# batmanlab/Mammo-CLIP

Measured on AMD Instinct MI355X. Metric: image-text pairs/s (whole node), EN-B5+BioClinicalBERT contrastive pre-training step, higher is better.
Workload: dtype bf16; 1 GPU; cfg4: efficientnet-b5 + BioClinicalBERT(BERT-base), 1024 pairs/GPU (2 views + 2 reports each), 1520x912 images, 256-token reports, breast_clip loss, AdamW; fwd+loss+bwd+optimizer; dropout/drop-connect on; global_batch=1024, parallelism=dp1 x 32 micro-batches, keep_graphs=7, recompute=0, keep_recompute=2, stat_tapes=True, streams=3

## Files before the change

include/mammoclip_hip.h:

```cpp
#ifndef MAMMOCLIP_HIP_H
#define MAMMOCLIP_HIP_H
#include <stdint.h>
#ifdef __cplusplus
extern "C" {
#endif

typedef uint16_t mc_bf16;

const char* mc_last_error(void);
int mc_version(void);
int mc_storage_is_f16(void);

typedef struct mc_gemm_args {
    const mc_bf16* A;
    const mc_bf16* B;
    void* C;
    long long M, K;
    int N;
    long long lda, ldb, ldc;
    int a_kmajor, b_kmajor;
    int c_f32, c_atomic;
    int splits;
    int batch, nb2;
    long long sA1, sA2, sB1, sB2, sC1, sC2;
// ... 57 lines not shown
    const float* epi_coef;
    const float* epi_mul;
    const float* epi_add;
    float epi_add_scale;
    float* epi_sums;
    float* epi_ws;
} mc_gemm_rows_args;
int mc_gemm_rows_supported(int n, int k);
long long mc_gemm_rows_epi_ws_floats(const mc_gemm_rows_args* args);
int mc_gemm_rows_epi_supported(long long M, int N, int K, long long rows_per_img, int epi_mode);
int mc_gemm_rows_blocks(const mc_gemm_rows_args* args);
int mc_gemm_rows_bf16(const mc_gemm_rows_args* args, void* stream);

typedef struct mc_wgrad_rows_args {
    const mc_bf16* dY;
    int N;
    long long lddy;
    const mc_bf16* X;
    int K;
    long long ldx;
    long long M;
    float* dW;
    float* ws;
    int accumulate;
    const float* pro_scale;
    const float* pro_shift;
    const float* pro_gate;
    long long pro_rows_per_img;
} mc_wgrad_rows_args;
int mc_wgrad_rows_supported(int n, int k);
int mc_wgrad_rows_blocks(long long m);
int mc_wgrad_rows_bf16(const mc_wgrad_rows_args* args, void* stream);
int mc_xbwd_rows_supported(int n, int k);
int mc_xbwd_rows_blocks(long long m);
int mc_xbwd_rows_bf16(const mc_wgrad_rows_args* args, const mc_bf16* wt, long long ldwt, mc_bf16* dx, long long lddx,
                      const mc_bf16* r, long long ldr, void* stream);

int mc_cast_f32_bf16(const float* src, mc_bf16* dst, long long n, void* stream);
int mc_cast_f32_bf16_lo(const float* src, mc_bf16* dst, long long n, void* stream);
int mc_cast_bf16_f32(const mc_bf16* src, float* dst, long long n, void* stream);
int mc_transpose_f32(const float* src, float* dst, int rows, int cols, void* stream);
int mc_cast_transpose_f32_bf16(const float* src, mc_bf16* dst, int rows, int cols, void* stream);
int mc_stem_weight_prep(const float* w, mc_bf16* out, int c0, void* stream);

int mc_stem_im2col(const float* x, long long sn, long long sc, long long sh, long long sw,
                   int n, int h, int w, int pad_l, int pad_t, int oh, int ow, mc_bf16* out, void* stream);
int mc_gate_weights_bf16(const mc_bf16* w, const float* gate, int n_img, int n, int k, mc_bf16* out, void* stream);

int mc_image_minmax_u8(const unsigned char* x, long long sn, long long elems_per_image, int n,
                       unsigned int* minmax, void* stream);
int mc_stem_im2col_u8(const unsigned char* x, long long sn, long long sc, long long sh, long long sw,
                      const unsigned int* minmax, float mean, float std, int n, int h, int w, int pad_l,
                      int pad_t, int oh, int ow, mc_bf16* out, void* stream);

typedef struct mc_dwconv_args {
    const mc_bf16* x;
    const mc_bf16* dy;
    void* out;
    const float* w_kkc;
    int n, h, w, c;
    int k, stride, pad_l, pad_t, oh, ow;
    const float* pro_scale;
    const float* pro_shift;
    float* stat_partials;
    const mc_bf16* epi_x;
    const float* epi_scale;
    const float* epi_shift;
    const float* epi_mean;
    const float* epi_invstd;
    float* dw_out;
    int stat_rows;
    const mc_bf16* xw;
    int cin;
    float* dw_partials;
    int dw_rows;
} mc_dwconv_args;
int mc_dwconv_stat_rows(const mc_dwconv_args* args);
int mc_dwconv_bwd_data_stat_rows(const mc_dwconv_args* args);
int mc_dwconv_fwd(const mc_dwconv_args* args, void* stream);
int mc_dwconv_bwd_data(const mc_dwconv_args* args, void* stream);
int mc_dwconv_bwd_weight(const mc_dwconv_args* args, void* stream);
int mc_dwconv_bwd_weight_dw_rows(const mc_dwconv_args* args);
int mc_dwconv_bwd_data_dw_rows(const mc_dwconv_args* args);
int mc_dwconv_bwd_fused_dw_rows(const mc_dwconv_args* args);
int mc_dwconv_bwd_data_xw_supported(const mc_dwconv_args* args);
int mc_dwconv_bwd_data_plan(const mc_dwconv_args* args, int* plan);
int mc_dwconv_bwd_data_xw_preferred(const mc_dwconv_args* args);
int mc_dwconv_set_lane_mode(int mode);
int mc_dwconv_lane_supported(const mc_dwconv_args* args);
int mc_dwconv_bwd_fused_supported(const mc_dwconv_args* args);
int mc_dwconv_bwd_fused_preferred(const mc_dwconv_args* args);
int mc_dwconv_bwd_fused_stat_rows(const mc_dwconv_args* args);
int mc_dwconv_bwd_fused(const mc_dwconv_args* args, void* stream);
int mc_mbconv_xdw_supported(const mc_dwconv_args* args);
int mc_mbconv_xdw_stat_rows(const mc_dwconv_args* args);
int mc_mbconv_xdw_fwd(const mc_dwconv_args* args, void* stream);

int mc_bn_finalize(const float* partials, int rows, int c, double count, const float* gamma,
                   const float* beta, float* running_mean, float* running_var, float momentum, float eps,
                   int update_running, float* mean, float* invstd, float* scale, float* shift, void* stream);
int mc_bn_eval_coeffs(const float* gamma, const float* beta, const float* running_mean,
                      const float* running_var, float eps, int c, float* scale, float* shift, void* stream);
int mc_bn_eval_stats(const float* gamma, const float* beta, const float* running_mean, const float* running_var,
                     float eps, int c, float* mean, float* invstd, float* scale, float* shift, void* stream);

typedef struct mc_bnact_args {
// ... 199 lines not shown
```

mammo_clip_amd/breastclip/model/modules/efficientnet_custom.py:

```python
import math
from collections import namedtuple
from typing import List, Optional

import os

import torch
from torch import nn

from .... import ops

BN_MOMENTUM = 0.01
BN_EPS = 1e-3

VALID_MODELS = tuple(f"efficientnet-b{i}" for i in range(9)) + ("efficientnet-l2",)

_COEFFS = {
    "efficientnet-b0": (1.0, 1.0, 224, 0.2), "efficientnet-b1": (1.0, 1.1, 240, 0.2),
    "efficientnet-b2": (1.1, 1.2, 260, 0.3), "efficientnet-b3": (1.2, 1.4, 300, 0.3),
    "efficientnet-b4": (1.4, 1.8, 380, 0.4), "efficientnet-b5": (1.6, 2.2, 456, 0.4),
    "efficientnet-b6": (1.8, 2.6, 528, 0.5), "efficientnet-b7": (2.0, 3.1, 600, 0.5),
    "efficientnet-b8": (2.2, 3.6, 672, 0.5), "efficientnet-l2": (4.3, 5.3, 800, 0.5),
}
_STAGES = ((1, 3, 1, 1, 32, 16), (2, 3, 2, 6, 16, 24), (2, 5, 2, 6, 24, 40), (3, 3, 2, 6, 40, 80),
           (3, 5, 1, 6, 80, 112), (4, 5, 2, 6, 112, 192), (1, 3, 1, 6, 192, 320))
# ... 99 lines not shown
            return
        if self.flat.is_cuda:
            self.flat.record_stream(torch.cuda.current_stream(self.flat.device))
        dst = [bn.running_mean for bn in self.used] + [bn.running_var for bn in self.used]
        src = [self.flat[self.offs[id(bn)]:self.offs[id(bn)] + bn.num_features] for bn in self.used] + \
              [self.flat[self.total + self.offs[id(bn)]:self.total + self.offs[id(bn)] + bn.num_features] for bn in self.used]
        torch._foreach_mul_(dst, 1.0 - BN_MOMENTUM)
        torch._foreach_add_(dst, src)
        self.used = []


_BN_DEFER = None


def _bn_stats(partials, count, bn: nn.BatchNorm2d, training: bool):
    if training:
        if _replaying():
            return _TAPE.get()
        if _BN_DEFER is not None and bn.track_update:
            rm, rv = _BN_DEFER.scratch(bn)
        else:
            rm, rv = bn.running_mean, bn.running_var
        st = ops.bn_finalize(partials, count, bn.weight, bn.bias, rm, rv, BN_MOMENTUM, BN_EPS, bn.track_update)
        if bn.track_update:
            if bn.defer_count is not None:
                bn.defer_count.append(bn.num_batches_tracked)
            else:
                bn.num_batches_tracked += 1
        if _TAPE is not None:
            _TAPE.put(st)
        return st
    return ops.bn_eval_coeffs(bn.weight, bn.bias, bn.running_mean, bn.running_var, BN_EPS)


def _conv_stats(fn, training, *a, stats=True, **kw):
    if not stats or (training and _replaying()):
        return fn(*a, **kw), None
    return fn(*a, stats=True, **kw)


def _no_fp8_frozen(mod):
    if mod.fp8:
        raise NotImplementedError("backward through BatchNorm on running statistics (eval mode / freeze_bn) is not implemented "
                                  "for the fp8 forward (set_fp8)")


LINK_STEM = os.environ.get("MC_LINK_STEM", "1") != "0"
FUSE_DW_BWD = os.environ.get("MC_FUSE_DW_BWD", "1") != "0"
FUSE_PROJ_DGRAD = os.environ.get("MC_FUSE_PROJ_DGRAD", "1") != "0"
BN_FOLD_MIN_BYTES = int(os.environ.get("MC_BN_FOLD_MIN_BYTES", 250_000_000))
BN_FOLD_S2_MIN_BYTES = int(os.environ.get("MC_BN_FOLD_S2_MIN_BYTES", 0))
XDW_MAX_CIN = int(os.environ.get("MC_XDW_MAX_CIN", 64))
MODE3_MAX_CEXP = int(os.environ.get("MC_MODE3_MAX_CEXP", 1 << 30))


class _StemFn(torch.autograd.Function):

    @staticmethod
    def forward(ctx, x, w, gamma, beta, mod, link=None):
        n, _, h, wd = x.shape
        l, r, t, b = mod.stem_pad
        _, oh, ow = mod.stem_geo(n, h, wd)
        c0 = w.shape[0]
        patches = ops.stem_im2col(x, l, t, oh, ow)
        wb = ops.stem_weight_prep(w)
        training = mod.batch_stats
        e, part = _conv_stats(ops.linear_fwd, training, patches, wb)
        st = _bn_stats(part, n * oh * ow, mod._bn0, training)
        ctx.mod, ctx.st, ctx.geo, ctx.frozen = mod, st, (n, h, wd, oh, ow, c0), not training
        ctx.raw = (x.mean, x.std) if isinstance(x, ops.RawImages) else None
        ctx.save_for_backward(x.data if ctx.raw else x, e)
        ctx.link = link
        if link is not None:
            link.st, link.part = st, None
            return e.detach()
        return ops.bnact_apply(e, n, oh * ow, c0, st.scale, st.shift, 1)

    @staticmethod
    def backward(ctx, dy):
        x, e = ctx.saved_tensors
        if ctx.raw:
            x = ops.RawImages(x, *ctx.raw)
        n, h, wd, oh, ow, c0 = ctx.geo
        mod = ctx.mod
        link = ctx.link
        if ctx.frozen:
            _no_fp8_frozen(mod)
        if ctx.frozen and link is not None:
            de = dy.contiguous()
            _, dgamma, dbeta = ops.bn_bwd_coefs(link.part, 0, ctx.st, mod._bn0.weight, frozen=True)
            link.part = None
        elif ctx.frozen:
            de, dgamma, dbeta = ops.bnact_bwd(e, n, oh * ow, c0, ctx.st, mod._bn0.weight, 1, g=dy.contiguous(), frozen=True)
        elif link is not None:
            de, dgamma, dbeta = ops.bnact_bwd(e, n, oh * ow, c0, ctx.st, mod._bn0.weight, 0, g=dy.contiguous(), partials=link.part)
            link.part = None
        else:
            de, dgamma, dbeta = ops.bnact_bwd(e, n, oh * ow, c0, ctx.st, mod._bn0.weight, 1, g=dy.contiguous())
        l, r, t, b = mod.stem_pad
        patches = ops.stem_im2col(x, l, t, oh, ow)
        dw = ops.linear_wgrad(de, patches)
        if ctx.frozen and link is not None:
            dw = ops.rowscale_f32_(dw, ctx.st.scale)
        gw, gg, gb = ops.deliver_param_grads((mod._conv_stem.weight, mod._bn0.weight, mod._bn0.bias),
                                             (dw[:, :27].reshape(c0, 3, 3, 3), dgamma, dbeta))
        return (None, gw, gg, gb, None) + ((None,) if link is not None else ())


class _StemLink:
    __slots__ = ("st", "part")

    def __init__(self):
        self.st, self.part = None, None


def _expand_conv(pl, x, we, stats=True):
    if pl.fp8_expand:
        return ops.linear_fwd_fp8(x, we, stats=True)
    return _conv_stats(ops.linear_fwd, pl.batch_stats, x, we, stats=stats)


def _depthwise(blk, pl, x, e, we, wkkc, pro0, stats=True):
    if pl.xdw:
        return _conv_stats(ops.mbconv_xdw_fwd, pl.batch_stats, x, we, pro0, wkkc, *pl.dw, stats=stats)
    return _conv_stats(ops.dwconv_fwd, pl.batch_stats, e if blk.args.expand != 1 else x, wkkc, *pl.dw, stats=stats, pro=pro0)


def _project_conv(pl, d, act1, st1, gate, wp, stats=True):
    ohw = pl.oh * pl.ow
    if pl.fp8_project:
        wg = ops.gate_weights(wp, gate)
        return ops.linear_fwd_fp8(act1, wg, stats=True, batch_w=(pl.n, ohw))
    src, pro = (act1, (None, None, gate, ohw)) if pl.keep_act else (d, (st1.scale, st1.shift, gate, ohw))
    return _conv_stats(ops.linear_fwd, pl.batch_stats, src, wp, stats=stats, pro=pro)


class _MBConvFn(torch.autograd.Function):

    @staticmethod
    def forward(ctx, x, rowscale, blk, n, h, w, recording, link, *params):
        a = blk.args
        pl = blk.plan(n, h, w, recording)
        training, bstat, ohw = pl.training, pl.batch_stats, pl.oh * pl.ow
        wkkc = blk.w_taps()
        e = we = st0 = gram = None
        if a.expand != 1:
            we = blk.w_expand()
            if pl.xdw:
                if bstat and _replaying():
                    part0, gram = None, _TAPE.get()
                elif bstat:
                    part0, gram = ops.bn_gram_partials(x, we, n * h * w)
# ... 598 lines not shown
```

mammo_clip_amd/lib.py:

```python
import ctypes as C
import os

_HERE = os.path.dirname(os.path.abspath(__file__))
STORAGE = os.environ.get("MC_STORAGE", "bf16").lower()
if STORAGE not in ("bf16", "f16"):
    raise ValueError(f"MC_STORAGE must be 'bf16' or 'f16', got {STORAGE!r}")
LIB_PATH = os.path.join(_HERE, "lib", "libmammoclip_hip.so" if STORAGE == "bf16" else "libmammoclip_hip_f16.so")

P, LL, I, F, D, U, ULL = C.c_void_p, C.c_longlong, C.c_int, C.c_float, C.c_double, C.c_uint, C.c_ulonglong


class GemmArgs(C.Structure):
    _fields_ = [
        ("A", P), ("B", P), ("C", P),
        ("M", LL), ("K", LL), ("N", I),
        ("lda", LL), ("ldb", LL), ("ldc", LL),
        ("a_kmajor", I), ("b_kmajor", I),
        ("c_f32", I), ("c_atomic", I),
        ("splits", I),
        ("batch", I), ("nb2", I),
        ("sA1", LL), ("sA2", LL), ("sB1", LL), ("sB2", LL), ("sC1", LL), ("sC2", LL),
        ("bias", P), ("bias_stride1", LL),
        ("act", I),
        ("R", P), ("ldr", LL),
# ... 52 lines not shown
        ("scale", P), ("shift", P), ("act", I),
        ("rowscale", P), ("res", P), ("out", P),
        ("pooled", P),
        ("g", P), ("mul", P), ("add", P), ("add_scale", F), ("mean", P), ("invstd", P),
        ("partials", P), ("coef", P), ("dx", P), ("dgate", P), ("split_ws", P),
    ]


class AdamwTensor(C.Structure):
    _fields_ = [("param", P), ("grad", P), ("exp_avg", P), ("exp_avg_sq", P), ("numel", LL), ("bf16_image", P)]


_SIGS = {
    "mc_version": ([], I),
    "mc_storage_is_f16": ([], I),
    "mc_adamw_step": ([C.POINTER(AdamwTensor), I, D, D, D, D, D, LL, P], I),
    "mc_grads_unscale": ([C.POINTER(AdamwTensor), I, F, P, P], I),
    "mc_grads_unscale_dev": ([C.POINTER(AdamwTensor), I, P, P, P], I),
    "mc_adamw_step_ls": ([C.POINTER(AdamwTensor), I, D, D, D, D, D, LL, P, P, P], I),
    "mc_loss_scale_update": ([P, P, D, D, I, I, P], I),
    "mc_grad_norm_partials": ([C.POINTER(AdamwTensor), I], LL),
    "mc_grad_norm": ([C.POINTER(AdamwTensor), I, P, LL, F, P, P], I),
    "mc_grads_unscale_norm_dev": ([C.POINTER(AdamwTensor), I, P, P, P, LL, F, P, P], I),
    "mc_grads_scale_dev": ([C.POINTER(AdamwTensor), I, P, P], I),
    "mc_adamw_step_clip": ([C.POINTER(AdamwTensor), I, D, D, D, D, D, LL, P, P, P, P], I),
    "mc_gemm_bf16": ([C.POINTER(GemmArgs), P], I),
    "mc_gemm_stat_rows": ([C.POINTER(GemmArgs)], I),
    "mc_gemm_tile_config": ([C.POINTER(GemmArgs)], I),
    "mc_gemm256_tn_eligible": ([C.POINTER(GemmArgs)], I),
    "mc_gemm256_tn_splits": ([LL, LL, LL, LL], I),
    "mc_amax_bf16": ([P, LL, P, P], I),
    "mc_quant_fp8_bf16": ([P, LL, P, P, P, P, P], I),
    "mc_gemm_rows_supported": ([I, I], I),
    "mc_gemm_rows_blocks": ([C.POINTER(GemmRowsArgs)], I),
    "mc_gemm_rows_epi_ws_floats": ([C.POINTER(GemmRowsArgs)], LL),
    "mc_gemm_rows_epi_supported": ([LL, I, I, LL, I], I),
    "mc_gemm_rows_bf16": ([C.POINTER(GemmRowsArgs), P], I),
    "mc_cast_transpose_f32_bf16": ([P, P, I, I, P], I),
    "mc_wgrad_rows_supported": ([I, I], I),
    "mc_wgrad_rows_blocks": ([LL], I),
    "mc_wgrad_rows_bf16": ([C.POINTER(WgradRowsArgs), P], I),
    "mc_xbwd_rows_supported": ([I, I], I),
    "mc_xbwd_rows_blocks": ([LL], I),
    "mc_xbwd_rows_bf16": ([C.POINTER(WgradRowsArgs), P, LL, P, LL, P, LL, P], I),
    "mc_cast_f32_bf16": ([P, P, LL, P], I),
    "mc_cast_bf16_f32": ([P, P, LL, P], I),
    "mc_cast_f32_bf16_lo": ([P, P, LL, P], I),
    "mc_transpose_f32": ([P, P, I, I, P], I),
    "mc_stem_weight_prep": ([P, P, I, P], I),
    "mc_stem_im2col": ([P, LL, LL, LL, LL, I, I, I, I, I, I, I, P, P], I),
    "mc_image_minmax_u8": ([P, LL, LL, I, P, P], I),
    "mc_gate_weights_bf16": ([P, P, I, I, I, P, P], I),
    "mc_stem_im2col_u8": ([P, LL, LL, LL, LL, P, F, F, I, I, I, I, I, I, I, P, P], I),
    "mc_dwconv_stat_rows": ([C.POINTER(DwconvArgs)], I),
    "mc_dwconv_bwd_data_stat_rows": ([C.POINTER(DwconvArgs)], I),
    "mc_dwconv_fwd": ([C.POINTER(DwconvArgs), P], I),
    "mc_dwconv_bwd_data": ([C.POINTER(DwconvArgs), P], I),
    "mc_dwconv_bwd_data_xw_supported": ([C.POINTER(DwconvArgs)], I),
    "mc_dwconv_bwd_data_plan": ([C.POINTER(DwconvArgs), C.POINTER(C.c_int)], I),
    "mc_dwconv_bwd_data_xw_preferred": ([C.POINTER(DwconvArgs)], I),
    "mc_dwconv_bwd_weight": ([C.POINTER(DwconvArgs), P], I),
    "mc_dwconv_bwd_weight_dw_rows": ([C.POINTER(DwconvArgs)], I),
    "mc_dwconv_bwd_data_dw_rows": ([C.POINTER(DwconvArgs)], I),
    "mc_dwconv_bwd_fused_dw_rows": ([C.POINTER(DwconvArgs)], I),
    "mc_dwconv_set_lane_mode": ([I], I),
    "mc_dwconv_lane_supported": ([C.POINTER(DwconvArgs)], I),
    "mc_dwconv_bwd_fused_supported": ([C.POINTER(DwconvArgs)], I),
    "mc_dwconv_bwd_fused_preferred": ([C.POINTER(DwconvArgs)], I),
    "mc_dwconv_bwd_fused_stat_rows": ([C.POINTER(DwconvArgs)], I),
    "mc_dwconv_bwd_fused": ([C.POINTER(DwconvArgs), P], I),
    "mc_mbconv_xdw_supported": ([C.POINTER(DwconvArgs)], I),
    "mc_mbconv_xdw_stat_rows": ([C.POINTER(DwconvArgs)], I),
    "mc_mbconv_xdw_fwd": ([C.POINTER(DwconvArgs), P], I),
    "mc_bn_gram_partials": ([P, I, P, P, D, I, I, P, P], I),
    "mc_bn_finalize": ([P, I, I, D, P, P, P, P, F, F, I, P, P, P, P, P], I),
    "mc_bn_eval_coeffs": ([P, P, P, P, F, I, P, P, P], I),
    "mc_bn_eval_stats": ([P, P, P, P, F, I, P, P, P, P, P], I),
    "mc_bnact_rows": ([C.POINTER(BnactArgs)], I),
    "mc_bnact_img_splits": ([C.POINTER(BnactArgs)], I),
    "mc_bnact_apply": ([C.POINTER(BnactArgs), P], I),
    "mc_bnact_pool": ([C.POINTER(BnactArgs), P], I),
    "mc_bnact_bwd_reduce": ([C.POINTER(BnactArgs), P], I),
    "mc_bnact_bwd_apply": ([C.POINTER(BnactArgs), P], I),
    "mc_bnact_bwd_frozen": ([C.POINTER(BnactArgs), P], I),
    "mc_bnact_se_dgate": ([C.POINTER(BnactArgs), P], I),
    "mc_bnact_se_sums": ([C.POINTER(BnactArgs), P], I),
    "mc_bn_partials_from_se_sums": ([P, P, P, F, LL, I, P, P], I),
    "mc_bn_bwd_finalize": ([P, I, I, D, P, P, P, P, P, P, P], I),
    "mc_bn_bwd_finalize_frozen": ([P, I, I, P, P, P, P, P], I),
    "mc_bn_frozen_rows": ([P, P, I, I, P, P, P], I),
    "mc_colsum_rows": ([LL, I], I),
    "mc_colsum_bf16": ([P, LL, I, LL, P, P, I, P], I),
    "mc_se_fwd": ([P, P, P, P, P, I, I, I, P, P, P], I),
    "mc_se_bwd": ([P, P, P, P, P, P, P, I, I, I, P, P, P, P, P, P, P], I),
    "mc_dropout_f32": ([P, P, LL, F, ULL, U, P], I),
    "mc_bert_embed_fwd": ([P, P, P, P, P, P, P, F, I, I, I, F, ULL, U, P, P, P, P], I),
    "mc_bert_embed_bwd": ([P, P, P, P, P, P, P, P, P, I, I, I, F, ULL, U, P, P, P, P, P, P], I),
    "mc_add_ln_fwd": ([P, P, P, P, F, LL, I, F, ULL, U, P, P, P, P], I),
    "mc_add_ln_bwd": ([P, P, P, P, P, P, LL, I, F, ULL, U, P, P, P, P, P], I),
    "mc_add_ln_bwd_ws_rows": ([LL], I),
    "mc_add_ln_bwd_ws": ([P, P, P, P, P, P, LL, I, F, ULL, U, P, P, P, P, P, I, P], I),
    "mc_bert_embed_bwd_ws_floats": ([I, I, I, LL, C.POINTER(C.c_int)], LL),
    "mc_bert_embed_bwd_ws": ([P, P, P, P, P, P, P, P, P, I, I, I, F, ULL, U, P, P, P, P, P, P, P, P, LL, P], I),
    "mc_ordered_sum": ([P, I, LL, LL, P, I, P], I),
    "mc_softmax_fwd": ([P, LL, I, F, ULL, U, P, P, P], I),
    "mc_softmax_bwd": ([P, P, LL, I, F, ULL, U, F, P, P], I),
# ... 122 lines not shown
```

mammo_clip_amd/ops.py:

```python
import ctypes as C
import math
import os

import weakref

import torch

from . import lib as L

BF16 = torch.bfloat16 if L.STORAGE == "bf16" else torch.float16


def _p(t):
    return None if t is None else t.data_ptr()


_RAW_STREAM = getattr(torch._C, "_cuda_getCurrentRawStream", None)
_GET_DEV = getattr(torch._C, "_cuda_getDevice", None)


def _st():
    if _RAW_STREAM is None or _GET_DEV is None:
        return torch.cuda.current_stream().cuda_stream
    return _RAW_STREAM(_GET_DEV())
# ... 497 lines not shown
        return dst
    return _cached("t", src, make) if cache else make()


def stem_weight_prep(w):
    c0 = w.shape[0]
    out = empty((c0, 32), BF16, w)
    L.call("mc_stem_weight_prep", _p(w.contiguous()), _p(out), c0, _st())
    return out


class RawImages:

    def __init__(self, data, mean, std):
        assert data.dtype == torch.uint8 and data.dim() == 4 and data.shape[1] == 3, "RawImages: uint8 [b,3,H,W]"
        self.data, self.mean, self.std = data, float(mean), float(std)

    def to(self, device, **kw):
        return RawImages(self.data.to(device, **kw), self.mean, self.std)

    shape = property(lambda self: self.data.shape)
    device = property(lambda self: self.data.device)
    is_cuda = property(lambda self: self.data.is_cuda)
    dtype = property(lambda self: self.data.dtype)


def image_minmax_u8(x):
    n = x.shape[0]
    per = x[0].numel()
    dense = sorted(zip(x.stride()[1:], x.shape[1:]), reverse=True)
    run = 1
    for st, sz in reversed(dense):
        assert sz == 1 or st == run, "RawImages: every image must be one dense block of bytes"
        run *= sz
    mm = torch.empty((2, n), dtype=torch.int32, device=x.device)
    L.call("mc_image_minmax_u8", _p(x), x.stride(0), per, n, _p(mm), _st())
    return mm


def stem_im2col(x, pad_l, pad_t, oh, ow):
    n, c, h, w = x.shape
    if isinstance(x, RawImages):
        d = x.data
        out = empty((n * oh * ow, 32), BF16, d)
        sn, sc, sh, sw = d.stride()
        L.call("mc_stem_im2col_u8", _p(d), sn, sc, sh, sw, _p(image_minmax_u8(d)), x.mean, x.std, n, h, w, pad_l, pad_t,
               oh, ow, _p(out), _st())
        return out
    assert c == 3 and x.dtype == torch.float32
    out = empty((n * oh * ow, 32), BF16, x)
    sn, sc, sh, sw = x.stride()
    L.call("mc_stem_im2col", _p(x), sn, sc, sh, sw, n, h, w, pad_l, pad_t, oh, ow, _p(out), _st())
    return out


def _dw_args(n, h, w, c, k, stride, pad_l, pad_t, oh, ow):
    a = L.DwconvArgs()
    a.n, a.h, a.w, a.c, a.k, a.stride, a.pad_l, a.pad_t, a.oh, a.ow = n, h, w, c, k, stride, pad_l, pad_t, oh, ow
    return a


def _dwconv_fwd_impl(x, w_kkc, n, h, w, c, k, stride, pad_l, pad_t, oh, ow, pro=None, stats=False, epi=None):
    a = _dw_args(n, h, w, c, k, stride, pad_l, pad_t, oh, ow)
    y = empty((n * oh * ow, c), BF16, x)
    a.x, a.out, a.w_kkc = _p(x), _p(y), _p(w_kkc)
    if pro is not None:
        a.pro_scale, a.pro_shift = _p(pro[0]), _p(pro[1])
    if epi is not None:
        e, st = epi
        assert stride == 1 and e.shape == y.shape
        a.epi_x, a.epi_scale, a.epi_shift, a.epi_mean, a.epi_invstd = _p(e), _p(st.scale), _p(st.shift), _p(st.mean), _p(st.invstd)
        stats = True
    part = None
    if stats:
        rows = L.load().mc_dwconv_stat_rows(C.byref(a))
        part = empty((rows, 2, c), torch.float32, x)
        a.stat_partials, a.stat_rows = _p(part), rows
    _note(2 * n * c * (h * w + oh * ow * (2 if epi is not None else 1)), 2 * n * c * oh * ow * k * k)
    L.call("mc_dwconv_fwd", C.byref(a), _st(), kind=f"k{k}s{stride}" + ("|dgrad_bn" if epi is not None else ""))
    return (y, part) if stats else y


def _dwconv_bwd_data_impl(dy, w_kkc, n, h, w, c, k, stride, pad_l, pad_t, oh, ow, w_kkc_flipped=None, epi=None, xw=None, dw=False):
    if stride == 1 and w_kkc_flipped is not None:
        assert xw is None and not dw
        return _dwconv_fwd_impl(dy, w_kkc_flipped, n, oh, ow, c, k, 1, k - 1 - pad_l, k - 1 - pad_t, h, w, epi=epi)
    assert epi is None or stride == 2
    if xw is not None:
        x, we = xw
        assert epi is not None and x.is_contiguous() and we.is_contiguous() and we.shape == (c, x.shape[1]) and x.shape[0] == n * h * w
        cin, st = x.shape[1], epi[1]
        a = _dw_args(n, h, w, c, k, stride, pad_l, pad_t, oh, ow)
        dz = empty((n * h * w, c), BF16, dy)
        a.dy, a.out, a.w_kkc = _p(dy), _p(dz), _p(w_kkc)
        a.epi_x, a.epi_scale, a.epi_shift, a.epi_mean, a.epi_invstd = _p(x), _p(st.scale), _p(st.shift), _p(st.mean), _p(st.invstd)
        a.xw, a.cin = _p(we), cin
        rows = L.load().mc_dwconv_bwd_data_stat_rows(C.byref(a))
        part = empty((rows, 2, c), torch.float32, dy)
        a.stat_partials, a.stat_rows = _p(part), rows
        dwdw = None
        if dw:
            dwdw = torch.zeros((k * k, c), dtype=torch.float32, device=dy.device)
            a.dw_out = _p(dwdw)
            ws = _dw_partials(a, "mc_dwconv_bwd_data_dw_rows", dy)
        _note(2 * n * (c * (oh * ow + h * w) + cin * h * w), (4 if dw else 2) * n * c * oh * ow * k * k + 2 * n * h * w * c * cin)
        L.call("mc_dwconv_bwd_data", C.byref(a), _st(), kind=f"k{k}s{stride}|dgrad_bn|x")
# ... 931 lines not shown
```

Before: 127.3 image-text pairs/s.

## Add direct stem convolution kernels fusing im2col, GEMM, BN stats and wgrad

Adds dedicated HIP kernels for the EfficientNet stem conv. The forward kernel loads image tiles (float or raw uint8 with normalisation) into LDS, runs MFMA against the weights and writes output plus BN statistic partials without materialising an im2col patch buffer. The backward kernel folds the BN-backward coefficients into a weight-gradient computation (dz·X and X·X Gram terms), so the separate bnact_bwd, im2col recompute and wgrad GEMM are skipped. By default the direct forward runs only outside training capture, while the direct backward runs whenever the BN is linked. This adds a multi-kernel reduction path and more numerical complexity in exchange.

```diff
diff --git a/include/mammoclip_hip.h b/include/mammoclip_hip.h
--- a/include/mammoclip_hip.h
+++ b/include/mammoclip_hip.h
@@ -133,6 +133,17 @@
 int mc_stem_im2col_u8(const unsigned char* x, long long sn, long long sc, long long sh, long long sw,
                       const unsigned int* minmax, float mean, float std, int n, int h, int w, int pad_l,
                       int pad_t, int oh, int ow, mc_bf16* out, void* stream);
+
+int mc_stem_conv_blocks(int n, int oh, int ow);
+int mc_stem_conv_set_max_blocks(int blocks);
+long long mc_stem_conv_bwd_ws_floats(int n, int oh, int ow, int c0);
+int mc_stem_conv_fwd(const void* x, int x_u8, long long sn, long long sc, long long sh, long long sw,
+                     const unsigned int* minmax, float mean, float std, int n, int h, int w, int pad_l, int pad_t,
+                     int oh, int ow, const mc_bf16* wimg, int c0, mc_bf16* e, float* stat_partials, void* stream);
+int mc_stem_conv_bwd(const void* x, int x_u8, long long sn, long long sc, long long sh, long long sw,
+                     const unsigned int* minmax, float mean, float std, int n, int h, int w, int pad_l, int pad_t,
+                     int oh, int ow, const mc_bf16* dz, const mc_bf16* wimg, const float* coef, int c0, float* ws,
+                     float* dw, void* stream);
 
 typedef struct mc_dwconv_args {
     const mc_bf16* x;
diff --git a/mammo_clip_amd/breastclip/model/modules/efficientnet_custom.py b/mammo_clip_amd/breastclip/model/modules/efficientnet_custom.py
--- a/mammo_clip_amd/breastclip/model/modules/efficientnet_custom.py
+++ b/mammo_clip_amd/breastclip/model/modules/efficientnet_custom.py
@@ -175,6 +175,7 @@
 BN_FOLD_S2_MIN_BYTES = int(os.environ.get("MC_BN_FOLD_S2_MIN_BYTES", 0))
 XDW_MAX_CIN = int(os.environ.get("MC_XDW_MAX_CIN", 64))
 MODE3_MAX_CEXP = int(os.environ.get("MC_MODE3_MAX_CEXP", 1 << 30))
+STEM_DIRECT = {"0": False, "1": True}.get(os.environ.get("MC_STEM_DIRECT", "1"), "all")
 
 
 class _StemFn(torch.autograd.Function):
@@ -185,12 +186,16 @@
         l, r, t, b = mod.stem_pad
         _, oh, ow = mod.stem_geo(n, h, wd)
         c0 = w.shape[0]
-        patches = ops.stem_im2col(x, l, t, oh, ow)
         wb = ops.stem_weight_prep(w)
         training = mod.batch_stats
-        e, part = _conv_stats(ops.linear_fwd, training, patches, wb)
+        direct = bool(STEM_DIRECT) and 24 <= c0 <= 64 and c0 % 8 == 0
+        if direct and (STEM_DIRECT == "all" or not (training and not _replaying())):
+            e, part = _conv_stats(ops.stem_conv_fwd, training, x, wb, l, t, oh, ow)
+        else:
+            e, part = _conv_stats(ops.linear_fwd, training, ops.stem_im2col(x, l, t, oh, ow), wb)
         st = _bn_stats(part, n * oh * ow, mod._bn0, training)
         ctx.mod, ctx.st, ctx.geo, ctx.frozen = mod, st, (n, h, wd, oh, ow, c0), not training
+        ctx.wb = wb if direct else None
         ctx.raw = (x.mean, x.std) if isinstance(x, ops.RawImages) else None
         ctx.save_for_backward(x.data if ctx.raw else x, e)
         ctx.link = link
@@ -209,6 +214,14 @@
         link = ctx.link
         if ctx.frozen:
             _no_fp8_frozen(mod)
+        l, r, t, b = mod.stem_pad
+        if ctx.wb is not None and link is not None:
+            coef, dgamma, dbeta = ops.bn_bwd_coefs(link.part, 0 if ctx.frozen else n * oh * ow, ctx.st, mod._bn0.weight, frozen=ctx.frozen)
+            link.part = None
+            dw = ops.stem_conv_bwd(x, dy.contiguous(), ctx.wb, coef, l, t, oh, ow)
+            gw, gg, gb = ops.deliver_param_grads((mod._conv_stem.weight, mod._bn0.weight, mod._bn0.bias),
+                                                 (dw[:, :27].reshape(c0, 3, 3, 3), dgamma, dbeta))
+            return (None, gw, gg, gb, None, None)
         if ctx.frozen and link is not None:
             de = dy.contiguous()
             _, dgamma, dbeta = ops.bn_bwd_coefs(link.part, 0, ctx.st, mod._bn0.weight, frozen=True)
@@ -220,7 +233,6 @@
             link.part = None
         else:
             de, dgamma, dbeta = ops.bnact_bwd(e, n, oh * ow, c0, ctx.st, mod._bn0.weight, 1, g=dy.contiguous())
-        l, r, t, b = mod.stem_pad
         patches = ops.stem_im2col(x, l, t, oh, ow)
         dw = ops.linear_wgrad(de, patches)
         if ctx.frozen and link is not None:
diff --git a/mammo_clip_amd/csrc/stem.hip b/mammo_clip_amd/csrc/stem.hip
--- /dev/null
+++ b/mammo_clip_amd/csrc/stem.hip
@@ -0,0 +1,449 @@
+#include "common_hip.h"
+#include "../../include/mammoclip_hip.h"
+
+namespace {
+
+typedef __attribute__((ext_vector_type(4))) short s4_t;
+typedef __attribute__((ext_vector_type(8))) short s8_t;
+typedef __attribute__((address_space(3))) s4_t lds_s4_t;
+
+constexpr int TW = 64, TR = 4;
+constexpr int IR = 2 * TR + 1;
+constexpr int IW = 2 * TW + 1;
+constexpr int PS = TW + 8;
+constexpr int NPL = IR * 9;
+constexpr int PL_ZERO = NPL, PL_ONE = NPL + 1;
+constexpr int SX_ELEMS = (NPL + 2) * PS;
+constexpr int RE = IW * 3;
+constexpr int NH = (RE + 255) / 256;
+constexpr int NLD = IR * NH;
+constexpr int MAX_BLOCKS = 768;
+
+struct stem_geo {
+    const void* x;
+    long long sn, sc, sh, sw;
+    int n, h, w, pad_l, pad_t, oh, ow, c0;
+    const unsigned int* mm;
+    float mean, stdv;
+    int tx, ty;
+    int ntiles;
+};
+
+struct tile_pos { long long img; int oy0, ox0; };
+__device__ __forceinline__ tile_pos tile_of(const stem_geo& g, int t) {
+    tile_pos q;
+    const unsigned t2 = (unsigned)t / (unsigned)g.tx, im = t2 / (unsigned)g.ty;
+    q.ox0 = (int)((unsigned)t - t2 * (unsigned)g.tx) * TW;
+    q.img = im;
+    q.oy0 = (int)(t2 - im * (unsigned)g.ty) * TR;
+    return q;
+}
+
+template <typename SRC>
+__device__ __forceinline__ void stem_load(const stem_geo& g, const tile_pos& q, int tid, SRC (&v)[NLD]) {
+    const int ix0 = q.ox0 * 2 - g.pad_l, iy0 = q.oy0 * 2 - g.pad_t;
+    const SRC* base = reinterpret_cast<const SRC*>(g.x) + q.img * g.sn;
+#pragma unroll
+    for (int hf = 0; hf < NH; ++hf) {
+        const int e = tid + hf * 256, ixl = e / 3, c = e - ixl * 3, ix = ix0 + ixl;
+        const int ixc = ix < 0 ? 0 : (ix < g.w ? ix : g.w - 1);
+        const long long xo = c * g.sc + ixc * g.sw;
+#pragma unroll
+        for (int r = 0; r < IR; ++r) {
+            const int iy = iy0 + r, iyc = iy < 0 ? 0 : (iy < g.h ? iy : g.h - 1);
+            v[r * NH + hf] = base[iyc * g.sh + xo];
+        }
+    }
+}
+
+template <typename SRC, bool MASK>
+__device__ __forceinline__ void stem_store(const stem_geo& g, const tile_pos& q, int tid, const SRC (&v)[NLD], bf16_t* sX) {
+    const int pvalid = MASK ? g.ow - q.ox0 : TW;
+    const int ix0 = q.ox0 * 2 - g.pad_l, iy0 = q.oy0 * 2 - g.pad_t;
+    float lo = 0.f, range = 1.f;
+    if constexpr (sizeof(SRC) == 1) {
+        lo = (float)g.mm[q.img];
+        range = (float)g.mm[g.n + q.img] - lo;
+    }
+#pragma unroll
+    for (int hf = 0; hf < NH; ++hf) {
+        const int e = tid + hf * 256, ixl = e / 3, c = e - ixl * 3, ix = ix0 + ixl;
+        const bool okx = ix >= 0 && ix < g.w;
+        const int p = ixl >> 1;
+        bf16_t* d0 = sX + c * 3 * PS + ((ixl & 1) ? PS + p : p);
+        bf16_t* d2 = sX + c * 3 * PS + 2 * PS + p - 1;
+        const bool w0 = e < RE && ((ixl & 1) || p < TW), w2 = e < RE && !(ixl & 1) && p >= 1;
+        const bool z0 = p >= pvalid, z2 = p - 1 >= pvalid;
+#pragma unroll
+        for (int r = 0; r < IR; ++r) {
+            const int iy = iy0 + r;
+            float val;
+            if constexpr (sizeof(SRC) == 1) {
+                float tt = (float)v[r * NH + hf] - lo;
+                tt = __fdiv_rn(tt, range);
+                val = __fdiv_rn(__fsub_rn(tt, g.mean), g.stdv);
+            } else {
+                val = v[r * NH + hf];
+            }
+            const bf16_t b = (okx && iy >= 0 && iy < g.h) ? f2bf(val) : (bf16_t)0;
+            if (w0) d0[r * 9 * PS] = z0 ? (bf16_t)0 : b;
+            if (w2) d2[r * 9 * PS] = z2 ? (bf16_t)0 : b;
+        }
+    }
+}
+
+__device__ __forceinline__ int plane_of(int k, int row, int pad27) {
+    if (k > 27) return PL_ZERO;
+    if (k == 27) return pad27;
+    const int cin = k / 9, kh = (k - cin * 9) / 3, kw = k - cin * 9 - kh * 3;
+    return (2 * row + kh) * 9 + cin * 3 + kw;
+}
+
+__device__ __forceinline__ bf16x8_t tr_read(const void* lo_addr, const void* hi_addr) {
+    const s4_t lo = __builtin_amdgcn_ds_read_tr16_b64_v4i16((lds_s4_t*)(lo_addr));
+    const s4_t hi = __builtin_amdgcn_ds_read_tr16_b64_v4i16((lds_s4_t*)(hi_addr));
+    const s8_t v = {lo[0], lo[1], lo[2], lo[3], hi[0], hi[1], hi[2], hi[3]};
+    return __builtin_bit_cast(bf16x8_t, v);
+}
+
+template <typename SRC, int FN>
+__global__ __launch_bounds__(256, 3) void stem_conv_fwd_k(const stem_geo g, const bf16_t* __restrict__ wimg, bf16_t* __restrict__ out,
+                                                       float* __restrict__ part) {
+    constexpr int NP = FN * 16, CROW = (NP + 8) * 2;
+    __shared__ __attribute__((aligned(16))) bf16_t sX[SX_ELEMS];
+    __shared__ __attribute__((aligned(16))) unsigned char sC[4 * 16 * CROW];
+    const int tid = threadIdx.x, lane = tid & 63, wave = tid >> 6;
+    const int li = lane & 15, kg = lane >> 4;
+    if (tid < PS) sX[PL_ZERO * PS + tid] = (bf16_t)0;
+
+    bf16x8_t wf[FN];
+#pragma unroll
+    for (int f = 0; f < FN; ++f) {
+        uint4 wv = make_uint4(0u, 0u, 0u, 0u);
+        if (f * 16 + li < g.c0) wv = *reinterpret_cast<const uint4*>(wimg + (f * 16 + li) * 32 + kg * 8);
+        wf[f] = __builtin_bit_cast(bf16x8_t, wv);
+    }
+    const bf16_t* bLo = sX + plane_of(kg * 8 + (li >> 2), wave, PL_ZERO) * PS + (li & 3) * 4;
+    const bf16_t* bHi = sX + plane_of(kg * 8 + 4 + (li >> 2), wave, PL_ZERO) * PS + (li & 3) * 4;
+
+    unsigned char* myC = sC + wave * 16 * CROW;
+    const int cpr = g.c0 >> 3;
+    const int slots = 64 / cpr;
+    const int c8 = lane % cpr, rs = lane / cpr;
+    const bool ep_active = rs < slots;
+    double dsum[8], dsq[8];
+#pragma unroll
+    for (int q = 0; q < 8; ++q) { dsum[q] = 0.0; dsq[q] = 0.0; }
+
+    SRC v[NLD];
+    int t = blockIdx.x;
+    stem_load<SRC>(g, tile_of(g, t), tid, v);
+    for (; t < g.ntiles; t += gridDim.x) {
+        const tile_pos tp = tile_of(g, t);
+        __syncthreads();
+        stem_store<SRC, false>(g, tp, tid, v, sX);
+        __syncthreads();
+        if (t + (int)gridDim.x < g.ntiles) stem_load<SRC>(g, tile_of(g, t + gridDim.x), tid, v);
+        const int oy = tp.oy0 + wave;
+        if (oy >= g.oh) continue;
+        const long long m0 = (tp.img * g.oh + oy) * g.ow + tp.ox0;
+        float ssum[8], ssq[8];
+#pragma unroll
+        for (int q = 0; q < 8; ++q) { ssum[q] = 0.f; ssq[q] = 0.f; }
+#pragma unroll
+        for (int gq = 0; gq < TW / 16; ++gq) {
+            const int p0 = gq * 16;
+            if (tp.ox0 + p0 >= g.ow) break;
+            const bf16x8_t xb = tr_read(bLo + p0, bHi + p0);
+#pragma unroll
+            for (int f = 0; f < FN; ++f) {
+                const f32x4_t acc = MC_MFMA_16x16x32(wf[f], xb, ((f32x4_t){0.f, 0.f, 0.f, 0.f}), 0, 0, 0);
+                const uint2 pk = make_uint2(pack_bf2(acc[0], acc[1]), pack_bf2(acc[2], acc[3]));
+                *reinterpret_cast<uint2*>(myC + li * CROW + (f * 16 + kg * 4) * 2) = pk;
+            }
+            __builtin_amdgcn_wave_barrier();
+            if (ep_active) {
+                for (int row = rs; row < 16; row += slots) {
+                    if (tp.ox0 + p0 + row < g.ow) {
+                        const uint4 ev = *reinterpret_cast<const uint4*>(myC + row * CROW + c8 * 16);
+                        if (part) {
+                            float a[8];
+                            unpack8(ev, a);
+#pragma unroll
+                            for (int q = 0; q < 8; ++q) { ssum[q] += a[q]; ssq[q] += a[q] * a[q]; }
+                        }
+                        *reinterpret_cast<uint4*>(out + (m0 + p0 + row) * g.c0 + c8 * 8) = ev;
+                    }
+                }
+            }
+            __builtin_amdgcn_wave_barrier();
+        }
+        if (part) {
+#pragma unroll
+            for (int q = 0; q < 8; ++q) { dsum[q] += (double)ssum[q]; dsq[q] += (double)ssq[q]; }
+        }
+    }
+
+    if (part) {
+        double* red = reinterpret_cast<double*>(sX);
+        double s = 0.0, s2 = 0.0;
+        for (int w = 0; w < 4; ++w) {
+            __syncthreads();
+            if (wave == w) {
+#pragma unroll
+                for (int q = 0; q < 8; ++q) {
+                    red[lane * 16 + q] = ep_active ? dsum[q] : 0.0;
+                    red[lane * 16 + 8 + q] = ep_active ? dsq[q] : 0.0;
+                }
+            }
+            __syncthreads();
+            if (tid < g.c0)
+                for (int r = 0; r < slots; ++r) {
+                    const double* e = red + (r * cpr + (tid >> 3)) * 16 + (tid & 7);
+                    s += e[0]; s2 += e[8];
+                }
+        }
+        if (tid < g.c0) {
+            float* dst = part + (long long)blockIdx.x * 4 * g.c0;
+            const float s_hi = (float)s, q_hi = (float)s2;
+            dst[tid] = s_hi; dst[g.c0 + tid] = q_hi;
+            dst[2 * g.c0 + tid] = (float)(s - (double)s_hi); dst[3 * g.c0 + tid] = (float)(s2 - (double)q_hi);
+        }
+    }
+}
+
+template <typename SRC, int FN>
+__global__ __launch_bounds__(256, 3) void stem_conv_bwd_k(const stem_geo g, const bf16_t* __restrict__ dz, float* __restrict__ ws) {
+    constexpr int NP = FN * 16, NR = NP + 32;
+    constexpr int DZ_BYTES = 4 * TW * NP * 2 + 64;
+    constexpr int SD_BYTES = DZ_BYTES > NR * 32 * 4 ? DZ_BYTES : NR * 32 * 4;
+    __shared__ __attribute__((aligned(16))) bf16_t sX[SX_ELEMS];
+    __shared__ __attribute__((aligned(16))) unsigned char sD[SD_BYTES];
+    const int tid = threadIdx.x, lane = tid & 63, wave = tid >> 6;
+    const int li = lane & 15, kg = lane >> 4;
+    if (tid < PS) sX[PL_ZERO * PS + tid] = (bf16_t)0;
+    const int rsy = g.c0 * 2;
+    unsigned char* myD = sD + wave * TW * rsy;
+    const bf16_t* pbase[2];
+#pragma unroll
+    for (int j = 0; j < 2; ++j) pbase[j] = sX + plane_of(j * 16 + li, wave, PL_ONE) * PS + kg * 8;
+
+    f32x4_t accG[FN][2], accS[2][2];
+#pragma unroll
+    for (int f = 0; f < FN; ++f)
+#pragma unroll
+        for (int j = 0; j < 2; ++j) accG[f][j] = (f32x4_t){0.f, 0.f, 0.f, 0.f};
+#pragma unroll
+    for (int i = 0; i < 2; ++i)
+#pragma unroll
+        for (int j = 0; j < 2; ++j) accS[i][j] = (f32x4_t){0.f, 0.f, 0.f, 0.f};
+
+    const int cpr = g.c0 >> 3;
+    uint4 dzr[2 * FN];
+    auto load_dz = [&](const tile_pos& tp) {
+        const int oy = tp.oy0 + wave < g.oh ? tp.oy0 + wave : g.oh - 1;
+        const long long m0 = (tp.img * g.oh + oy) * g.ow;
+#pragma unroll
+        for (int j = 0; j < 2 * FN; ++j) {
+            const int ch = lane + j * 64, px = ch / cpr, cc = ch - px * cpr;
+            const int ox = tp.ox0 + px < g.ow ? tp.ox0 + px : g.ow - 1;
+            if (j < cpr) dzr[j] = *reinterpret_cast<const uint4*>(dz + (m0 + ox) * g.c0 + cc * 8);
+        }
+    };
+    auto store_dz = [&](const tile_pos& tp) {
+        const bool oky = tp.oy0 + wave < g.oh;
+#pragma unroll
+        for (int j = 0; j < 2 * FN; ++j) {
+            const int ch = lane + j * 64, px = ch / cpr, cc = ch - px * cpr;
+            if (j < cpr)
+                *reinterpret_cast<uint4*>(myD + px * rsy + cc * 16) = oky && tp.ox0 + px < g.ow ? dzr[j] : make_uint4(0u, 0u, 0u, 0u);
+        }
+    };
+
+    SRC v[NLD];
+    int t = blockIdx.x;
+    {
+        const tile_pos first = tile_of(g, t);
+        stem_load<SRC>(g, first, tid, v);
+        load_dz(first);
+    }
+    for (; t < g.ntiles; t += gridDim.x) {
+        const tile_pos tp = tile_of(g, t);
+        __syncthreads();
+        stem_store<SRC, true>(g, tp, tid, v, sX);
+        store_dz(tp);
+        if (tid < TW) sX[PL_ONE * PS + tid] = tp.ox0 + tid < g.ow ? f2bf(1.f) : (bf16_t)0;
+        __syncthreads();
+        if (t + (int)gridDim.x < g.ntiles) {
+            const tile_pos nxt = tile_of(g, t + gridDim.x);
+            stem_load<SRC>(g, nxt, tid, v);
+            load_dz(nxt);
+        }
+        if (tp.oy0 + wave >= g.oh) continue;
+#pragma unroll
+        for (int ks = 0; ks < TW / 32; ++ks) {
+            const int p0 = ks * 32;
+            if (tp.ox0 + p0 >= g.ow) break;
+            bf16x8_t a[FN], pb[2];
+#pragma unroll
+            for (int f = 0; f < FN; ++f) {
+                const unsigned char* ad = myD + (p0 + kg * 8 + (li >> 2)) * rsy + (f * 16 + (li & 3) * 4) * 2;
+                a[f] = tr_read(ad, ad + 4 * rsy);
+            }
+#pragma unroll
+            for (int j = 0; j < 2; ++j) pb[j] = *reinterpret_cast<const bf16x8_t*>(pbase[j] + p0);
+#pragma unroll
+            for (int f = 0; f < FN; ++f)
+#pragma unroll
+                for (int j = 0; j < 2; ++j) accG[f][j] = MC_MFMA_16x16x32(a[f], pb[j], accG[f][j], 0, 0, 0);
+#pragma unroll
+            for (int i = 0; i < 2; ++i)
+#pragma unroll
+                for (int j = 0; j < 2; ++j) accS[i][j] = MC_MFMA_16x16x32(pb[i], pb[j], accS[i][j], 0, 0, 0);
+        }
+    }
+
+    float* red = reinterpret_cast<float*>(sD);
+    for (int w = 0; w < 4; ++w) {
+        __syncthreads();
+        if (wave != w) continue;
+#pragma unroll
+        for (int fr = 0; fr < FN + 2; ++fr)
+#pragma unroll
+            for (int j = 0; j < 2; ++j)
+#pragma unroll
+                for (int r = 0; r < 4; ++r) {
+                    const float val = fr < FN ? accG[fr < FN ? fr : 0][j][r] : accS[fr < FN ? 0 : fr - FN][j][r];
+                    float* d = red + (fr * 16 + kg * 4 + r) * 32 + j * 16 + li;
+                    *d = w == 0 ? val : *d + val;
+                }
+    }
+    __syncthreads();
+    float* dst = ws + (long long)blockIdx.x * NR * 32;
+    for (int i = tid; i < NR * 32; i += 256) dst[i] = red[i];
+}
+
+__global__ __launch_bounds__(256) void stem_bwd_reduce_k(const float* __restrict__ ws, int parts, int ne, double* __restrict__ sums) {
+    __shared__ double sh[16][17];
+    const int el = threadIdx.x & 15, pl = threadIdx.x >> 4;
+    const int i = blockIdx.x * 16 + el;
+    double s = 0.0;
+    if (i < ne)
+        for (int k = pl; k < parts; k += 16) s += (double)ws[(long long)k * ne + i];
+    sh[pl][el] = s;
+    __syncthreads();
+    if (pl != 0 || i >= ne) return;
+    s = 0.0;
+    for (int k = 0; k < 16; ++k) s += sh[k][el];
+    sums[i] = s;
+}
+
+__global__ __launch_bounds__(256) void stem_bwd_finish_k(const double* __restrict__ sums, int np, const bf16_t* __restrict__ wimg,
+                                                         const float* __restrict__ coef, int c0, float* __restrict__ dw) {
+    const int idx = blockIdx.x * 256 + threadIdx.x;
+    if (idx >= c0 * 32) return;
+    const int o = idx >> 5, k = idx & 31;
+    double r = 0.0;
+    if (k < 27) {
+        const double* S = sums + (long long)np * 32;
+        double ws_ = 0.0;
+        for (int j = 0; j < 27; ++j) ws_ += (double)bf2f(wimg[o * 32 + j]) * S[j * 32 + k];
+        r = (double)coef[o] * sums[o * 32 + k] + (double)coef[c0 + o] * ws_ + (double)coef[2 * c0 + o] * S[27 * 32 + k];
+    }
+    dw[idx] = (float)r;
+}
+
+int g_max_blocks = MAX_BLOCKS;
+
+int make_geo(stem_geo& g, const void* x, long long sn, long long sc, long long sh, long long sw, int n, int h, int w, int pad_l,
+             int pad_t, int oh, int ow, int c0) {
+    g.x = x; g.sn = sn; g.sc = sc; g.sh = sh; g.sw = sw;
+    g.n = n; g.h = h; g.w = w; g.pad_l = pad_l; g.pad_t = pad_t; g.oh = oh; g.ow = ow; g.c0 = c0;
+    g.mm = nullptr; g.mean = 0.f; g.stdv = 1.f;
+    g.tx = (ow + TW - 1) / TW; g.ty = (oh + TR - 1) / TR;
+    const long long nt = (long long)n * g.tx * g.ty;
+    g.ntiles = (int)(nt < (1LL << 30) ? nt : 0);
+    return g.ntiles < g_max_blocks ? g.ntiles : g_max_blocks;
+}
+
+template <typename SRC> int launch_fwd(const stem_geo& g, int blocks, const bf16_t* wimg, bf16_t* out, float* part, hipStream_t st) {
+    switch ((g.c0 + 15) / 16) {
+        case 2: hipLaunchKernelGGL((stem_conv_fwd_k<SRC, 2>), dim3(blocks), dim3(256), 0, st, g, wimg, out, part); break;
+        case 3: hipLaunchKernelGGL((stem_conv_fwd_k<SRC, 3>), dim3(blocks), dim3(256), 0, st, g, wimg, out, part); break;
+        default: hipLaunchKernelGGL((stem_conv_fwd_k<SRC, 4>), dim3(blocks), dim3(256), 0, st, g, wimg, out, part); break;
+    }
+    MC_LAUNCH_CHECK();
+    return MC_OK;
+}
+
+template <typename SRC> int launch_bwd(const stem_geo& g, int blocks, const bf16_t* dz, const bf16_t* wimg, const float* coef,
+                                       float* ws, float* dw, hipStream_t st) {
+    const int np = (g.c0 + 15) / 16 * 16, ne = (np + 32) * 32;
+    switch (np / 16) {
+        case 2: hipLaunchKernelGGL((stem_conv_bwd_k<SRC, 2>), dim3(blocks), dim3(256), 0, st, g, dz, ws); break;
+        case 3: hipLaunchKernelGGL((stem_conv_bwd_k<SRC, 3>), dim3(blocks), dim3(256), 0, st, g, dz, ws); break;
+        default: hipLaunchKernelGGL((stem_conv_bwd_k<SRC, 4>), dim3(blocks), dim3(256), 0, st, g, dz, ws); break;
+    }
+    MC_LAUNCH_CHECK();
+    double* sums = reinterpret_cast<double*>(ws + (long long)blocks * ne);
+    hipLaunchKernelGGL(stem_bwd_reduce_k, dim3(mc_div_up(ne, 16)), dim3(256), 0, st, ws, blocks, ne, sums);
+    MC_LAUNCH_CHECK();
+    hipLaunchKernelGGL(stem_bwd_finish_k, dim3(mc_div_up(g.c0 * 32, 256)), dim3(256), 0, st, sums, np, wimg, coef, g.c0, dw);
+    MC_LAUNCH_CHECK();
+    return MC_OK;
+}
+
+bool geo_ok(int n, int h, int w, int pad_l, int pad_t, int oh, int ow, int c0) {
+    return (long long)n * ((ow + TW - 1) / TW) * ((oh + TR - 1) / TR) < (1LL << 30) && n > 0 && h > 0 && w > 0 && oh > 0 && ow > 0 && pad_l >= 0 && pad_t >= 0 && c0 >= 24 && c0 <= 64 && c0 % 8 == 0;
+}
+
+}
+
+extern "C" int mc_stem_conv_set_max_blocks(int blocks) {
+    MC_CHECK(blocks >= 0 && blocks <= MAX_BLOCKS, "stem_conv_set_max_blocks: 0 (default) .. 768");
+    g_max_blocks = blocks ? blocks : MAX_BLOCKS;
+    return MC_OK;
+}
+
+extern "C" int mc_stem_conv_blocks(int n, int oh, int ow) {
+    if (n <= 0 || oh <= 0 || ow <= 0) return 0;
+    stem_geo g;
+    return make_geo(g, nullptr, 0, 0, 0, 0, n, 1, 1, 0, 0, oh, ow, 32);
+}
+
+extern "C" long long mc_stem_conv_bwd_ws_floats(int n, int oh, int ow, int c0) {
+    const long long ne = ((c0 + 15) / 16 * 16 + 32) * 32;
+    return (long long)mc_stem_conv_blocks(n, oh, ow) * ne + 2 * ne;
+}
+
+extern "C" int mc_stem_conv_fwd(const void* x, int x_u8, long long sn, long long sc, long long sh, long long sw,
+                                const unsigned int* minmax, float mean, float std, int n, int h, int w, int pad_l, int pad_t,
+                                int oh, int ow, const mc_bf16* wimg, int c0, mc_bf16* e, float* stat_partials, void* stream) {
+    MC_CHECK(x && wimg && e && geo_ok(n, h, w, pad_l, pad_t, oh, ow, c0), "stem_conv_fwd: bad args (c0 in 24..64, a multiple of 8)");
+    MC_CHECK(!x_u8 || (minmax && std != 0.f), "stem_conv_fwd: the uint8 source needs minmax and a non-zero std");
+    MC_CHECK(mc_aligned16(e) && mc_aligned16(wimg), "stem_conv_fwd: e and the weight image must be 16-byte aligned");
+    stem_geo g;
+    const int blocks = make_geo(g, x, sn, sc, sh, sw, n, h, w, pad_l, pad_t, oh, ow, c0);
+    if (x_u8) {
+        g.mm = minmax; g.mean = mean; g.stdv = std;
+        return launch_fwd<unsigned char>(g, blocks, (const bf16_t*)wimg, (bf16_t*)e, stat_partials, (hipStream_t)stream);
+    }
+    return launch_fwd<float>(g, blocks, (const bf16_t*)wimg, (bf16_t*)e, stat_partials, (hipStream_t)stream);
+}
+
+extern "C" int mc_stem_conv_bwd(const void* x, int x_u8, long long sn, long long sc, long long sh, long long sw,
+                                const unsigned int* minmax, float mean, float std, int n, int h, int w, int pad_l, int pad_t,
+                                int oh, int ow, const mc_bf16* dz, const mc_bf16* wimg, const float* coef, int c0, float* ws,
+                                float* dw, void* stream) {
+    MC_CHECK(x && dz && wimg && coef && ws && dw && geo_ok(n, h, w, pad_l, pad_t, oh, ow, c0),
+             "stem_conv_bwd: bad args (c0 in 24..64, a multiple of 8)");
+    MC_CHECK(!x_u8 || (minmax && std != 0.f), "stem_conv_bwd: the uint8 source needs minmax and a non-zero std");
+    MC_CHECK(mc_aligned16(dz) && ((((uintptr_t)ws) & 7u) == 0), "stem_conv_bwd: dz must be 16-byte, the workspace 8-byte aligned");
+    stem_geo g;
+    const int blocks = make_geo(g, x, sn, sc, sh, sw, n, h, w, pad_l, pad_t, oh, ow, c0);
+    if (x_u8) {
+        g.mm = minmax; g.mean = mean; g.stdv = std;
+        return launch_bwd<unsigned char>(g, blocks, (const bf16_t*)dz, (const bf16_t*)wimg, coef, ws, dw, (hipStream_t)stream);
+    }
+    return launch_bwd<float>(g, blocks, (const bf16_t*)dz, (const bf16_t*)wimg, coef, ws, dw, (hipStream_t)stream);
+}
diff --git a/mammo_clip_amd/lib.py b/mammo_clip_amd/lib.py
--- a/mammo_clip_amd/lib.py
+++ b/mammo_clip_amd/lib.py
@@ -128,6 +128,11 @@
     "mc_image_minmax_u8": ([P, LL, LL, I, P, P], I),
     "mc_gate_weights_bf16": ([P, P, I, I, I, P, P], I),
     "mc_stem_im2col_u8": ([P, LL, LL, LL, LL, P, F, F, I, I, I, I, I, I, I, P, P], I),
+    "mc_stem_conv_blocks": ([I, I, I], I),
+    "mc_stem_conv_set_max_blocks": ([I], I),
+    "mc_stem_conv_bwd_ws_floats": ([I, I, I, I], LL),
+    "mc_stem_conv_fwd": ([P, I, LL, LL, LL, LL, P, F, F, I, I, I, I, I, I, I, P, I, P, P, P], I),
+    "mc_stem_conv_bwd": ([P, I, LL, LL, LL, LL, P, F, F, I, I, I, I, I, I, I, P, P, P, I, P, P, P], I),
     "mc_dwconv_stat_rows": ([C.POINTER(DwconvArgs)], I),
     "mc_dwconv_bwd_data_stat_rows": ([C.POINTER(DwconvArgs)], I),
     "mc_dwconv_fwd": ([C.POINTER(DwconvArgs), P], I),
diff --git a/mammo_clip_amd/ops.py b/mammo_clip_amd/ops.py
--- a/mammo_clip_amd/ops.py
+++ b/mammo_clip_amd/ops.py
@@ -573,6 +573,46 @@
     sn, sc, sh, sw = x.stride()
     L.call("mc_stem_im2col", _p(x), sn, sc, sh, sw, n, h, w, pad_l, pad_t, oh, ow, _p(out), _st())
     return out
+
+
+def _stem_src(x):
+    if isinstance(x, RawImages):
+        return x.data, 1, image_minmax_u8(x.data), x.mean, x.std
+    assert x.shape[1] == 3 and x.dtype == torch.float32
+    return x, 0, None, 0.0, 1.0
+
+
+def stem_conv_set_max_blocks(blocks):
+    L.call("mc_stem_conv_set_max_blocks", int(blocks))
+
+
+def stem_conv_fwd(x, wb, pad_l, pad_t, oh, ow, stats=False):
+    d, u8, mm, mean, std = _stem_src(x)
+    _chk_dev(d, wb)
+    n, _, h, w = d.shape
+    c0 = wb.shape[0]
+    e = empty((n * oh * ow, c0), BF16, d)
+    part = empty((2 * L.load().mc_stem_conv_blocks(n, oh, ow), 2, c0), torch.float32, d) if stats else None
+    sn, sc, sh, sw = d.stride()
+    _note(d.numel() * d.element_size() + 2 * n * oh * ow * c0)
+    L.call("mc_stem_conv_fwd", _p(d), u8, sn, sc, sh, sw, _p(mm), mean, std, n, h, w, pad_l, pad_t, oh, ow, _p(wb), c0, _p(e),
+           _p(part), _st())
+    return (e, part) if stats else e
+
+
+def stem_conv_bwd(x, dz, wb, coef, pad_l, pad_t, oh, ow):
+    d, u8, mm, mean, std = _stem_src(x)
+    _chk_dev(d, dz, wb, coef)
+    n, _, h, w = d.shape
+    c0 = wb.shape[0]
+    assert dz.shape == (n * oh * ow, c0) and dz.is_contiguous() and coef.shape == (3, c0) and coef.is_contiguous()
+    ws = empty((L.load().mc_stem_conv_bwd_ws_floats(n, oh, ow, c0),), torch.float32, d)
+    dw = empty((c0, 32), torch.float32, d)
+    sn, sc, sh, sw = d.stride()
+    _note(2 * n * oh * ow * c0 + d.numel() * d.element_size())
+    L.call("mc_stem_conv_bwd", _p(d), u8, sn, sc, sh, sw, _p(mm), mean, std, n, h, w, pad_l, pad_t, oh, ow, _p(dz), _p(wb),
+           _p(coef), c0, _p(ws), _p(dw), _st())
+    return dw
 
 
 def _dw_args(n, h, w, c, k, stride, pad_l, pad_t, oh, ow):
```

Measured after the change: 128.4 image-text pairs/s, median of 6. About the same (+0.9%).
